# utiasDSL/upright

Measured on AMD Instinct MI355X. Metric: batched MPC solves/sec + ms/SQP-iter, Thing 1-obj horizon=20, 1/2/4/8 GPU, higher is better.
Workload: dtype f64

## Files before the change

### __graft_entry__.py

```python
import os
import subprocess
import sys
from pathlib import Path

ROOT = Path(__file__).resolve().parent
CSRC = ROOT / "upright_amd" / "csrc"
LIB = ROOT / "upright_amd" / "libupright_mi.so"


def _newer(srcs, out):
    return (not out.exists()) or any(s.stat().st_mtime > out.stat().st_mtime for s in srcs)


def n_qp3_parts():
    import re

    m = re.search(r"#define\s+UPR_QP3_NPARTS\s+(\d+)", (CSRC / "upr_qp3_list.h").read_text())
    return int(m.group(1))


def build_engine(out=None, extra_flags=()):
    from concurrent.futures import ThreadPoolExecutor

    out = Path(out) if out else LIB
# ... 42 lines not shown
        subprocess.check_call(["g++", "-O2", "-std=c++17", "-fPIC", "-shared", "-Wno-unknown-pragmas", "-o", str(bal_out), str(bal_src)])
    mar_src = ROOT / "tests" / "emu" / "upr_margin_emu.cpp"
    mar_out = ROOT / "tests" / "emu" / "libupr_margin_emu.so"
    if _newer(srcs + [mar_src], mar_out):
        subprocess.check_call(["g++", "-O2", "-std=c++17", "-fPIC", "-shared", "-Wno-unknown-pragmas", "-o", str(mar_out), str(mar_src)])
    grp_src = ROOT / "tests" / "emu" / "upr_group_margin_emu.cpp"
    grp_out = ROOT / "tests" / "emu" / "libupr_group_margin_emu.so"
    if _newer(srcs + [grp_src], grp_out):
        subprocess.check_call(["g++", "-O2", "-std=c++17", "-fPIC", "-shared", "-Wno-unknown-pragmas", "-o", str(grp_out), str(grp_src)])
    spd_src = ROOT / "tests" / "emu" / "upr_speed_emu.cpp"
    spd_out = ROOT / "tests" / "emu" / "libupr_speed_emu.so"
    if _newer(srcs + [spd_src], spd_out):
        subprocess.check_call(["g++", "-O2", "-std=c++17", "-fPIC", "-shared", "-Wno-unknown-pragmas", "-o", str(spd_out), str(spd_src)])
    spd_fma = ROOT / "tests" / "emu" / "libupr_speed_emu_fma.so"
    if has_fma and _newer(srcs + [spd_src], spd_fma):
        subprocess.check_call(["g++", "-O2", "-mfma", "-ffp-contract=fast", "-std=c++17", "-fPIC", "-shared", "-Wno-unknown-pragmas", "-o", str(spd_fma), str(spd_src)])
    pac_src = ROOT / "tests" / "emu" / "upr_pathacc_emu.cpp"
    pac_out = ROOT / "tests" / "emu" / "libupr_pathacc_emu.so"
    if _newer(srcs + [pac_src], pac_out):
        subprocess.check_call(["g++", "-O2", "-std=c++17", "-fPIC", "-shared", "-Wno-unknown-pragmas", "-o", str(pac_out), str(pac_src)])
    pac_fma = ROOT / "tests" / "emu" / "libupr_pathacc_emu_fma.so"
    if has_fma and _newer(srcs + [pac_src], pac_fma):
        subprocess.check_call(["g++", "-O2", "-mfma", "-ffp-contract=fast", "-std=c++17", "-fPIC", "-shared", "-Wno-unknown-pragmas", "-o", str(pac_fma), str(pac_src)])
    sys.path.insert(0, str(ROOT))
    import upright_amd
    from upright_amd import _capi

    _capi.lib()


def smoke():
    import json

    import numpy as np

    sys.path.insert(0, str(ROOT))
    from oracle.oracle import Oracle
    from upright_amd.engine import BatchMPC
    from upright_amd.problem import thing_problem
    from upright_amd.sampling import level_tray_states, stationary_guess, waypoints_for

    arr = json.load(open(ROOT / "tests" / "golden" / "arrangements.json"))["pink_bottle"]
    P = thing_problem(arr)
    B = 4
    x0 = level_tray_states(B, seed=3)
    way = waypoints_for(P, x0)
# ... 21 lines not shown
```

### upright_amd/csrc/upr_api.hip

```cpp
#include <hip/hip_runtime.h>
#include <hip/hiprtc.h>

#include <dlfcn.h>
#include <sys/stat.h>
#include <unistd.h>

#include <algorithm>
#include <chrono>
#include <fstream>
#include <map>
#include <mutex>
#include <sstream>
#include <cmath>
#include <cstdio>
#include <cstdlib>
#include <cstring>
#include <string>
#include <vector>

#include "upr_common.h"
#include "upr_kin.h"
#include "upr_linearize.h"
#include "upr_linearize2.h"
#include "upr_linesearch.h"
#include "upr_qp.h"
#include "upr_qp2.h"
#include "upr_qp3.h"
#include "upr_qp3_list.h"
#include "upr_qp3_launch.h"
#include "upr_qp_select.h"
#include "upr_launch_select.h"
#include "upr_value.h"
#include "upr_balance.h"
#include "upr_margin.h"
#include "upr_speed.h"
#include "upr_pathacc.h"
#include "upr_iface.h"

namespace {

thread_local std::string g_err;

int fail(const std::string& msg) {
    g_err = msg;
    return 1;
}

#define UPR_HIP(call)                                                                                 \
    do {                                                                                              \
        hipError_t e_ = (call);                                                                       \
        if (e_ != hipSuccess) return fail(std::string(#call) + ": " + hipGetErrorString(e_) + " (upr_api.hip:" + std::to_string(__LINE__) + ")"); \
    } while (0)

// ... 67 lines not shown
    if (threadIdx.x == 0) done[b] = 0;
}

__global__ void evaluate_kernel(const upr_problem* P, upr_dims d, int B, const double* tsol, const double* xs,
                                const double* us, const double* t, int t_stride, double* x_out, double* u_out) {
    int b = blockIdx.x;
    const int N = d.N, nx = d.nx, nu = d.nu;
    const double tau = t[(size_t)b * t_stride];
    for (int i = threadIdx.x; i < nx; i += blockDim.x)
        upr_interp(d, P->dt, tsol[b], xs + (size_t)b * (N + 1) * nx, us + (size_t)b * N * nu, tau, i, 0, x_out + (size_t)b * nx + i, nullptr);
    for (int i = threadIdx.x; i < nu; i += blockDim.x)
        upr_interp(d, P->dt, tsol[b], xs + (size_t)b * (N + 1) * nx, us + (size_t)b * N * nu, tau, 0, i, nullptr, u_out + (size_t)b * nu + i);
}

struct upr_fb_src {
    int kind;
    long k_base; int k_stride;
    long lji_base; int lji_stride;
    long lfi_base; int lfi_stride;
    long lsi_base; int lsi_stride;
    int lsi_sb;
};

template <int NEM, int NFM>
__global__ void feedback_kernel(const upr_problem* P, upr_dims d, upr_fb_src src, const double* ws, const double* lin,
                                const double* Df, const double* stats, double* fb) {
    const int b = blockIdx.x;
    const int N = d.N, nq = d.nq, nx = d.nx, nu = d.nu, ne = d.ne, nfc = d.nfc, nf = d.nf;
    const double* w = ws + (size_t)b * d.ws_stride;
    double* out = fb + (size_t)b * N * nu * nx;
    if (stats[(size_t)b * UPR_NSTATS + 2] == 2.0) {
        for (int e = threadIdx.x; e < N * nu * nx; e += blockDim.x) out[e] = 0.0;
        return;
    }
    for (int e = threadIdx.x; e < N * nq * nx; e += blockDim.x) {
        const int k = e / (nq * nx), j = (e % (nq * nx)) / nx, c = e % nx;
        double v;
        if (src.kind == 3) v = w[src.k_base + (long)k * src.k_stride + j * nx + c];
        else {
            const double* V = w + src.k_base + (long)k * src.k_stride;
            const double* Lji = w + src.lji_base + (long)k * src.lji_stride;
            v = 0.0;
            for (int m = j; m < nq; ++m) v += Lji[m * nq + j] * V[m * nx + c];
        }
        out[((size_t)k * nu + j) * nx + c] = -v;
    }
    const double* Dfb = Df + (size_t)b * ne * nfc;
    for (int e = threadIdx.x; e < N * nx; e += blockDim.x) {
        const int k = e / nx, c = e % nx;
        const double* Ck = lin + ((size_t)b * (N + 1) + k) * d.lin_stride + d.lin_gx;
        const double* Lsi = w + src.lsi_base + (long)k * src.lsi_stride;
        const double* Lfi = w + src.lfi_base + (long)k * src.lfi_stride;
        double t1[NEM], t2[NEM], t3[NFM];
        const int sb = src.lsi_sb;
        for (int r = 0; r < ne; ++r) { const int b0 = (r / sb) * sb; const double* Lb = Lsi + (b0 / sb) * sb * sb; double v = 0.0; for (int m = b0; m <= r; ++m) v += Lb[(r - b0) * sb + (m - b0)] * Ck[m * nx + c]; t1[r] = v; }
        for (int r = 0; r < ne; ++r) { const int b0 = (r / sb) * sb; const double* Lb = Lsi + (b0 / sb) * sb * sb; double v = 0.0; for (int m = r; m < b0 + sb; ++m) v += Lb[(m - b0) * sb + (r - b0)] * t1[m]; t2[r] = v; }
        for (int i = 0; i < nfc; ++i) { double v = 0.0; for (int r = 0; r < ne; ++r) v += Dfb[r * nfc + i] * t2[r]; t3[i] = v; }
        for (int ci = 0; ci < d.nc; ++ci) {
            if (nf == 3) {
                const double* Bk = Lfi + 9 * ci; const double* x3 = t3 + 3 * ci;
                double y[3], z[3];
                for (int a = 0; a < 3; ++a) { double v = 0.0; for (int b2 = 0; b2 <= a; ++b2) v += Bk[3 * a + b2] * x3[b2]; y[a] = v; }
                for (int a = 0; a < 3; ++a) { double v = 0.0; for (int b2 = a; b2 < 3; ++b2) v += Bk[3 * b2 + a] * y[b2]; z[a] = v; }
                for (int a = 0; a < 3; ++a) out[((size_t)k * nu + nq + 3 * ci + a) * nx + c] = -z[a];
            } else {
                const double lf = Lfi[ci];
                out[((size_t)k * nu + nq + ci) * nx + c] = -lf * lf * t3[ci];
            }
        }
    }
}

__global__ void evaluate_policy_kernel(const upr_problem* P, upr_dims d, int B, const double* tsol, const double* xs,
                                       const double* us, const double* fb, const double* t, const double* x_obs,
                                       double* x_out, double* u_out) {
    const int b = blockIdx.x;
    const int N = d.N, nx = d.nx, nu = d.nu;
    const double* X = xs + (size_t)b * (N + 1) * nx; const double* U = us + (size_t)b * N * nu;
    const double* K = fb + (size_t)b * N * nu * nx; const double* xo = x_obs + (size_t)b * nx;
    double s = (t[b] - tsol[b]) / P->dt;
    if (s < 0.0) s = 0.0;
    for (int i = threadIdx.x; i < nx; i += blockDim.x)
        upr_interp(d, P->dt, tsol[b], X, U, t[b], i, 0, x_out + (size_t)b * nx + i, nullptr);
    for (int i = threadIdx.x; i < nu; i += blockDim.x) {
        double v = 0.0;
        if (s <= N) {
            int j = (int)s; if (j > N - 1) j = N - 1;
            const double a = (s >= N - 1) ? 0.0 : s - j;
            const int j1 = (j + 1 < N) ? j + 1 : N - 1;
            double v0 = U[j * nu + i], v1 = U[j1 * nu + i];
            for (int c = 0; c < nx; ++c) {
                v0 += K[((size_t)j * nu + i) * nx + c] * (xo[c] - X[j * nx + c]);
                if (a > 0.0) v1 += K[((size_t)j1 * nu + i) * nx + c] * (xo[c] - X[j1 * nx + c]);
            }
            v = (1.0 - a) * v0 + a * v1;
        }
        u_out[(size_t)b * nu + i] = v;
    }
}

}

#define UPR_ENTER(h) do { if (!(h)) return fail("null batch"); if ((h)->device >= 0) UPR_HIP(hipSetDevice((h)->device)); } while (0)

struct upr_jit_kernel {
    hipModule_t mod = nullptr;
    hipFunction_t fn = nullptr;
    size_t lds = 0, ws = 0;
    int nt = 256;
    std::string cfg;
    upr_fb_src fb{};
};

struct upr_qp_sel : upr_qp_choice {
    int (*launch)(struct upr_batch*, const upr_qp_args&) = nullptr;
    upr_jit_kernel* jit = nullptr;
    upr_fb_src fb{};
};

struct upr_lin_sel : upr_lin_choice {
    const void* kern = nullptr;
    char name[128] = "";
};
// ... 12 lines not shown
struct upr_stats_snapshot {
    std::vector<double> stats; std::vector<unsigned char> keys;
};
}

struct upr_batch {
    upr_problem P;
    upr_dims d;
    int B = 0;
    int device = -1;
    hipStream_t stream = nullptr;
    upr_problem* dP = nullptr;
    double *body_params = nullptr, *way_p = nullptr, *way_q = nullptr, *t0 = nullptr, *x0 = nullptr;
    double *xs = nullptr, *us = nullptr, *xs_prev = nullptr, *us_prev = nullptr, *tprev = nullptr;
    double *lin = nullptr, *Df = nullptr, *ws = nullptr, *stats = nullptr;
    int *done = nullptr;
    bool has_prev = false;
    unsigned char* iter_key = nullptr;
    int* order = nullptr;
    bool order_on = true, order_valid = false;
    double* prof = nullptr;
    double *ev_t = nullptr, *ev_xo = nullptr, *ev_x = nullptr, *ev_u = nullptr;
    double* kkt = nullptr;
    double *fb = nullptr, *xs_lin = nullptr;
    double *dyn0 = nullptr, *pflag = nullptr;
    std::vector<double> hdyn0, hdyn_prev;
    double* pin = nullptr;
    hipGraphExec_t tick_exec = nullptr;
    unsigned long long tick_sig = 0;
    int tick_steady = 0;
    int tick_graph_on = -1;
    long long tick_replays = 0;
    int nxf = 0;
    bool guess_set = false;
    int sqp_iters_next = 0;
    double last_ms = 0.0;
    upr_qp_sel qp;
    upr_lin_sel lin_sel;
    upr_ls_sel ls_sel;
    int lin_blocks_last = -1;
    bool ls_launched = false;
    int timing = 0;
    unsigned timing_qp_count = 0;
    double k_ms[3] = {0, 0, 0};
    int k_launches[3] = {0, 0, 0};
    std::vector<double> hDf;
// ... 358 lines not shown
    void stop() { if (on) (void)hipEventRecord(h->ev_pool[idx + 1], h->stream); }
};

int vf_alloc(upr_batch* h) {
    if (h->vf_P) return 0;
    const size_t B = (size_t)h->B, n1 = (size_t)h->d.N + 1, nx = (size_t)h->d.nx;
    if (dev_alloc(&h->vf_P, B * n1 * nx * nx) || dev_alloc(&h->vf_p, B * n1 * nx) || dev_alloc(&h->vf_J, B * n1) || dev_alloc(&h->vf_X, B * n1 * nx) || dev_alloc(&h->vf_t0, B) ||
        dev_alloc(&h->vf_nu, B * (size_t)h->d.N * (size_t)h->d.ne)) return 1;
    UPR_HIP(hipEventCreate(&h->vf_ev[0])); UPR_HIP(hipEventCreate(&h->vf_ev[1]));
    return 0;
}
upr_vf_args make_vf_args(upr_batch* h) {
    upr_vf_args A;
    A.P = h->dP; A.d = h->d; A.xs = h->xs; A.us = h->us; A.lin = h->lin; A.Df = h->Df; A.ws = h->ws;
    const upr_qp_sel& q = h->qp;
    A.mult = q.exported ? h->kkt : h->ws; A.mult_stride = q.stride;
    A.o_pi = q.o_pi; A.o_nu = q.o_nu; A.o_lam = q.o_lam; A.o_t = q.o_t; A.o_sig = q.o_sig; A.o_tau = q.o_tau; A.o_gam = q.o_gam;
    A.Pk = h->vf_P; A.pk = h->vf_p; A.J = h->vf_J; A.X = h->vf_X; A.nu_out = h->vf_nu;
    return A;
}
size_t vf_lds_bytes(const upr_batch* h) { return (size_t)upr_vf_lds_layout(h->d).total * sizeof(double); }
hipError_t vf_raise_lds_limit() { return hipFuncSetAttribute((const void*)upr_value_kernel, hipFuncAttributeMaxDynamicSharedMemorySize, 160 * 1024); }

int advance_impl(upr_batch* h) {
    const upr_dims& d = h->d;
    if (h->vf_state) h->vf_state = 2;
    if (!h->guess_set) {
        hipLaunchKernelGGL(prepare_kernel, dim3(h->B), dim3(256), 0, h->stream, h->dP, d, h->B, h->has_prev ? 1 : 0, h->tprev,
                           h->xs_prev, h->us_prev, h->t0, h->x0, h->xs, h->us, h->stats, h->done);
        UPR_HIP(hipGetLastError());
    } else {
        UPR_HIP(hipMemsetAsync(h->stats, 0, sizeof(double) * h->B * UPR_NSTATS, h->stream));
        UPR_HIP(hipMemsetAsync(h->done, 0, sizeof(int) * h->B, h->stream));
        h->guess_set = false;
    }
    const int sqp_iters = h->sqp_iters_next > 0 ? h->sqp_iters_next : h->P.sqp_iters;
    h->sqp_iters_next = 0;
    for (int it = 0; it < sqp_iters; ++it) {
        { KernelTimer T(h, 0); if (launch_linearize(h, traj_lin_args(h))) return 1; T.stop(); }
        {
            upr_qp_args Q = make_qp_args(h);
            if (h->fb && h->qp.fb_fused && it == sqp_iters - 1) Q.fb = h->fb;
            if (h->order_on && h->order_valid) Q.order = h->order;
            if (h->vf_track && it == sqp_iters - 1 && h->qp.exported) { Q.kkt = h->kkt; Q.kkt_stride = h->qp.stride; }
            KernelTimer T(h, 1); if (launch_qp(h, Q)) return 1; T.stop();
        }
        if (h->vf_track && it == sqp_iters - 1) {
            const bool timed = h->timing != 0;
            if (timed) UPR_HIP(hipEventRecord(h->vf_ev[0], h->stream));
            hipLaunchKernelGGL(upr_value_kernel, dim3(h->B), dim3(UPR_VF_NT), vf_lds_bytes(h), h->stream, make_vf_args(h));
            UPR_HIP(hipGetLastError());
            if (timed) { UPR_HIP(hipEventRecord(h->vf_ev[1], h->stream)); h->vf_ms_pending = true; }
            UPR_HIP(hipMemcpyAsync(h->vf_t0, h->t0, sizeof(double) * h->B, hipMemcpyDeviceToDevice, h->stream));
            h->vf_state = 1; h->vf_tracked = true;
        }
        upr_ls_args L;
        L.P = h->dP; L.d = d; L.xs = h->xs; L.us = h->us; L.x0 = h->x0; L.t0 = h->t0; L.body_params = h->body_params;
        L.way_p = h->way_p; L.way_q = upr_has_orientation_cost(&h->P) ? h->way_q : nullptr; L.lin = h->lin; L.ws = h->ws; L.stats = h->stats; L.done = h->done; L.iter = it; L.dyn = h->dyn0; L.pflag = h->pflag;
        if (h->order_on) { L.order_out = h->order; L.iter_key = h->iter_key; }
        if (it == sqp_iters - 1) { L.xs_prev = h->xs_prev; L.us_prev = h->us_prev; L.tprev = h->tprev; }
        { KernelTimer T(h, 2); if (launch_linesearch(h, L)) return 1; T.stop(); }
        if (h->order_on) h->order_valid = true;
    }
    if (h->fb && !(h->qp.fb_fused && sqp_iters > 0)) {
        if (h->qp.fb.kind == 0) return fail("feedback gains: the selected QP kernel names no source for them");
        if (d.ne <= 6 && d.nfc <= 12) hipLaunchKernelGGL((feedback_kernel<6, 12>), dim3(h->B), dim3(256), 0, h->stream, h->dP, d, h->qp.fb, h->ws, h->lin, h->Df, h->stats, h->fb);
        else hipLaunchKernelGGL((feedback_kernel<6 * UPR_MAX_BODIES, 3 * UPR_MAX_CONTACTS>), dim3(h->B), dim3(256), 0, h->stream, h->dP, d, h->qp.fb, h->ws, h->lin, h->Df, h->stats, h->fb);
        UPR_HIP(hipGetLastError());
    }
    h->hdyn_prev = h->hdyn0;
    if (sqp_iters <= 0) {
        UPR_HIP(hipMemcpyAsync(h->xs_prev, h->xs, sizeof(double) * h->B * (d.N + 1) * d.nx, hipMemcpyDeviceToDevice, h->stream));
        UPR_HIP(hipMemcpyAsync(h->us_prev, h->us, sizeof(double) * h->B * d.N * d.nu, hipMemcpyDeviceToDevice, h->stream));
        UPR_HIP(hipMemcpyAsync(h->tprev, h->t0, sizeof(double) * h->B, hipMemcpyDeviceToDevice, h->stream));
    }
    h->has_prev = true;
    return 0;
}

enum { BAL_MU_NONE = 0, BAL_MU_SCENARIO = 1, BAL_MU_CONTACT = 2 };
enum { BAL_RHO = 0, BAL_MARGIN = 1, BAL_MARGIN_GROUPS = 2, BAL_SPEED = 3, BAL_PATHACC = 4 };
struct bal_request {
    const char* who = "";
    const char* needs = "";
    bool plan = false; int n = 0; const double* x = nullptr;
    int n_scen = 0; const double* params = nullptr; bool per = false;
    int scale = BAL_MU_NONE; const double* mu_scale = nullptr;
    int quantity = BAL_RHO; double kappa_max = 0.0; int n_grp = 1; const unsigned* group_mask = nullptr; const double* mu_base = nullptr;
    double s_max = 0.0; double* limit = nullptr;
    double d_max = 0.0, speed = 1.0;
    double* out = nullptr;
    double *kappa_lo = nullptr, *z = nullptr, *y = nullptr; int* iters = nullptr; double* worst = nullptr; int* worst_knot = nullptr;
// ... 235 lines not shown
    UPR_HIP(hipMemcpy(out, dout, sizeof(double) * n * 5 * P->nc, hipMemcpyDeviceToHost));
    return 0;
}

upr_batch* upr_batch_create(const upr_problem* P, int B, const double* body_params, const double* way_p) {
    if (check_problem(P)) return nullptr;
    if (B < 1) { fail("B must be >= 1"); return nullptr; }
    if (need_device()) return nullptr;
    upr_batch* h = new upr_batch();
    if (hipGetDevice(&h->device) != hipSuccess) { fail("hipGetDevice failed"); delete h; return nullptr; }
    h->P = *P; h->d = upr_make_dims(P); h->B = B;
    h->nxf = (int)upr_iface_width(h->d.nx, P->n_dyn);
    h->hdyn0.assign((size_t)B * upr_iface_dyn_width(P->n_dyn), 0.0); h->hdyn_prev = h->hdyn0;
    const upr_dims& d = h->d;
    if (d.nx > UPR_LPK) { fail("nx exceeds the 32 tangent lanes of the linearisation kernel"); delete h; return nullptr; }
    {
        upr_qp_knobs k;
        if (const char* e = getenv("UPR_QP_KERNEL")) k.qp_kernel = atoi(e);
        if (const char* e = getenv("UPR_QP_GENERIC")) k.qp_generic = atoi(e) != 0;
        if (const char* e = getenv("UPR_QP3_JIT")) k.qp3_jit = atoi(e);
        if (const char* e = getenv("UPR_QP_NT")) { k.qp_nt_set = true; k.qp_nt = atoi(e); }
        if (const char* e = getenv("UPR_QP_GENERIC_NT")) { k.generic_nt_set = true; k.generic_nt = atoi(e); }
        if (const char* e = getenv("UPR_JIT_NT")) k.jit_nt = atoi(e);
        if (const char* e = getenv("UPR_FB_FUSED")) k.fb_fused = atoi(e) != 0;
        upr_qp_sel& s = h->qp;
        static_cast<upr_qp_choice&>(s) = upr_qp_plan(*P, d, k);
        if (s.source == UPR_QP_FROM_RUN_TIME && s.structure == UPR_QP_STRUCT_PRODUCTION && jit_get(s.cfg, s.nt, &s.jit) != 0) {
            static_cast<upr_qp_choice&>(s) = upr_qp_plan(*P, d, k, false);
            fprintf(stderr, "libupright_mi: %s -- using the %s kernel instead\n", g_err.c_str(), s.structure == UPR_QP_STRUCT_SECOND ? "second-structure" : "generic");
        }
        qp_resolve(s, *P, d);
        h->d.ws_stride = s.ws_stride;
    }
    {
        upr_lin_knobs kl; upr_ls_knobs ks;
        if (const char* e = getenv("UPR_LIN_MFMA")) kl.mfma = atoi(e) != 0;
        if (const char* e = getenv("UPR_LIN2")) kl.lin2 = atoi(e) != 0;
        if (const char* e = getenv("UPR_LIN_OCC")) kl.occ = atoi(e);
        if (const char* e = getenv("UPR_LIN_ROW_PASSES")) kl.row_passes = atoi(e);
        if (const char* e = getenv("UPR_LS_STAGE_FULL")) ks.stage_full = atoi(e);
        static_cast<upr_lin_choice&>(h->lin_sel) = upr_lin_plan(*P, d, kl);
        static_cast<upr_ls_choice&>(h->ls_sel) = upr_ls_plan(*P, d, ks);
        h->lin_sel.kern = (P->nq == 6) ? lin_kernel<6>(h->lin_sel) : lin_kernel<9>(h->lin_sel);
        h->ls_sel.kern = (P->nq == 6) ? ls_kernel<6>(h->ls_sel) : ls_kernel<9>(h->ls_sel);
        upr_ls_name(h->ls_sel, h->ls_sel.name, sizeof(h->ls_sel.name));
        if (!h->lin_sel.kern || !h->ls_sel.kern) { fail("the planned linearisation / line-search form is not an instantiation of upr_launch_select.h's lists"); delete h; return nullptr; }
    }
    if (const char* e = getenv("UPR_QP_ORDER")) h->order_on = atoi(e) != 0;
    {
        const char* e = getenv("UPR_BAL_FORM");
        h->bal.L = upr_bal_layout(d.nb, d.nc, d.nf);
        h->bal.lds = (size_t)h->bal.L.total * sizeof(double);
        h->bal.form = (upr_bal_lane_form(d.nb) && !(e && atoi(e) == 0)) ? BAL_LANE : BAL_WAVE;
    }
    auto bad = [&]() { upr_batch_destroy(h); return (upr_batch*)nullptr; };
    if (hipStreamCreate(&h->stream) != hipSuccess) { fail("hipStreamCreate failed"); return bad(); }
    if (hipMalloc((void**)&h->dP, sizeof(upr_problem)) != hipSuccess) { fail("hipMalloc failed"); return bad(); }
    hipMemcpy(h->dP, P, sizeof(upr_problem), hipMemcpyHostToDevice);
    const size_t n1 = d.N + 1;
    if (dev_alloc(&h->body_params, (size_t)B * d.nb * 10) || dev_alloc(&h->way_p, (size_t)B * P->n_way * 3) || dev_alloc(&h->way_q, (size_t)B * P->n_way * 4) ||
        dev_alloc(&h->t0, (((size_t)B + 1) & ~(size_t)1) + (size_t)B * d.nx + (size_t)B * upr_iface_dyn_width(P->n_dyn)) || dev_alloc(&h->xs, (size_t)B * n1 * d.nx) || dev_alloc(&h->us, (size_t)B * d.N * d.nu) ||
        dev_alloc(&h->xs_prev, (size_t)B * n1 * d.nx) || dev_alloc(&h->us_prev, (size_t)B * d.N * d.nu) || dev_alloc(&h->tprev, B) ||
        dev_alloc(&h->lin, (size_t)B * n1 * d.lin_stride) || dev_alloc(&h->Df, (size_t)B * d.ne * d.nfc) ||
        dev_alloc(&h->ws, (size_t)B * d.ws_stride) || dev_alloc(&h->stats, (size_t)B * UPR_NSTATS) || dev_alloc(&h->done, B) || dev_alloc(&h->order, B) || dev_alloc(&h->iter_key, ((size_t)B + 3) & ~(size_t)3) ||
        (P->use_feedback_policy && dev_alloc(&h->fb, (size_t)B * d.N * d.nu * d.nx)) ||
        (P->n_dyn && dev_alloc(&h->pflag, B)))
        return bad();
    h->x0 = h->t0 + (((size_t)B + 1) & ~(size_t)1);
    if (P->n_dyn) h->dyn0 = h->x0 + (size_t)B * d.nx;
    hipMemcpy(h->body_params, body_params, sizeof(double) * B * d.nb * 10, hipMemcpyHostToDevice);
    hipMemcpy(h->way_p, way_p, sizeof(double) * B * P->n_way * 3, hipMemcpyHostToDevice);
    {
        std::vector<double> qi((size_t)B * P->n_way * 4, 0.0);
        for (size_t i = 3; i < qi.size(); i += 4) qi[i] = 1.0;
        hipMemcpy(h->way_q, qi.data(), sizeof(double) * qi.size(), hipMemcpyHostToDevice);
    }
    h->hDf.assign((size_t)B * d.ne * d.nfc, 0.0);
    std::vector<double> unit(d.nfc), Fw(6 * d.nb);
    const double scale = 1.0 / std::sqrt(6.0 * d.nb);
    for (int b = 0; b < B; ++b) {
        const double* bp = body_params + (size_t)b * d.nb * 10;
        for (int j = 0; j < d.nfc; ++j) {
            std::fill(unit.begin(), unit.end(), 0.0);
            unit[j] = 1.0;
            upr_object_wrenches(P, bp, unit.data(), Fw.data());
            for (int bb = 0; bb < d.nb; ++bb)
                for (int r = 0; r < 6; ++r) h->hDf[((size_t)b * d.ne + 6 * bb + r) * d.nfc + j] = -scale * Fw[6 * bb + r] / bp[10 * bb];
        }
// ... 86 lines not shown
int upr_batch_advance(upr_batch* h) {
    UPR_ENTER(h);
    auto t0 = std::chrono::steady_clock::now();
    if (advance_impl(h)) return 1;
    UPR_HIP(hipStreamSynchronize(h->stream));
    h->last_ms = std::chrono::duration<double, std::milli>(std::chrono::steady_clock::now() - t0).count();
    return 0;
}

static int get_solution_core(upr_batch* h, double* ts, double* xs, double* us) {
    const upr_dims& d = h->d;
    UPR_HIP(hipStreamSynchronize(h->stream));
    if (ts) {
        std::vector<double> t0(h->B);
        UPR_HIP(hipMemcpy(t0.data(), h->t0, sizeof(double) * h->B, hipMemcpyDeviceToHost));
        for (int b = 0; b < h->B; ++b) for (int k = 0; k <= d.N; ++k) ts[(size_t)b * (d.N + 1) + k] = t0[b] + k * h->P.dt;
    }
    if (xs) UPR_HIP(hipMemcpy(xs, h->xs, sizeof(double) * h->B * (d.N + 1) * d.nx, hipMemcpyDeviceToHost));
    if (us) UPR_HIP(hipMemcpy(us, h->us, sizeof(double) * h->B * d.N * d.nu, hipMemcpyDeviceToHost));
    return 0;
}

static int evaluate_core(upr_batch* h, const double* t, int t_stride, bool policy, const double* x_obs, double* x_out, double* u_out) {
    if (policy && !h->fb) return fail("upr_batch_evaluate_policy: the batch was created with use_feedback_policy = 0");
    const upr_dims& d = h->d;
    if (eval_scratch(h)) return 1;
    std::vector<double> tt(h->B);
    instance_times(h->B, t, t_stride, tt.data());
    UPR_HIP(hipMemcpyAsync(h->ev_t, tt.data(), sizeof(double) * h->B, hipMemcpyHostToDevice, h->stream));
    if (policy) {
        UPR_HIP(hipMemcpyAsync(h->ev_xo, x_obs, sizeof(double) * h->B * d.nx, hipMemcpyHostToDevice, h->stream));
        hipLaunchKernelGGL(evaluate_policy_kernel, dim3(h->B), dim3(64), 0, h->stream, h->dP, d, h->B, h->tprev, h->xs_prev, h->us_prev, h->fb, h->ev_t, h->ev_xo, h->ev_x, h->ev_u);
    } else hipLaunchKernelGGL(evaluate_kernel, dim3(h->B), dim3(64), 0, h->stream, h->dP, d, h->B, h->tprev, h->xs_prev, h->us_prev, h->ev_t, 1, h->ev_x, h->ev_u);
    UPR_HIP(hipGetLastError());
    UPR_HIP(hipMemcpyAsync(x_out, h->ev_x, sizeof(double) * h->B * d.nx, hipMemcpyDeviceToHost, h->stream));
    UPR_HIP(hipMemcpyAsync(u_out, h->ev_u, sizeof(double) * h->B * d.nu, hipMemcpyDeviceToHost, h->stream));
    UPR_HIP(hipStreamSynchronize(h->stream));
    return 0;
}

static int get_feedback_core(upr_batch* h, double* K) {
    if (!h->fb) return fail("upr_batch_get_feedback: the batch was created with use_feedback_policy = 0");
    const upr_dims& d = h->d;
    UPR_HIP(hipStreamSynchronize(h->stream));
    UPR_HIP(hipMemcpy(K, h->fb, sizeof(double) * h->B * d.N * d.nu * d.nx, hipMemcpyDeviceToHost));
    return 0;
}

double upr_batch_last_solve_ms(const upr_batch* h) { return h ? h->last_ms : 0.0; }

const char* upr_batch_qp_kernel_name(const upr_batch* h) { return h ? h->qp.name : ""; }

const char* upr_batch_ls_kernel_name(upr_batch* h) {
    if (!h || !h->ls_launched) return "";
    return h->ls_sel.name;
}

const char* upr_batch_lin_kernel_name(upr_batch* h) {
    if (!h || h->lin_blocks_last < 0) return "";
    upr_lin_name(h->lin_sel, h->lin_blocks_last, h->lin_sel.name, sizeof(h->lin_sel.name));
    return h->lin_sel.name;
}

int upr_batch_hold_stats(upr_batch* h, int restore) {
    UPR_ENTER(h);
    UPR_HIP(hipStreamSynchronize(h->stream));
    if (!restore) return snapshot_take(h, h->held);
    if (h->held.stats.empty()) return fail("upr_batch_hold_stats: nothing held on this handle");
    if (snapshot_put_back(h, h->held)) return 1;
    h->held = upr_stats_snapshot();
    return 0;
}

int upr_batch_get_stats(upr_batch* h, double* stats) {
    UPR_ENTER(h);
    UPR_HIP(hipStreamSynchronize(h->stream));
    UPR_HIP(hipMemcpy(stats, h->stats, sizeof(double) * h->B * UPR_NSTATS, hipMemcpyDeviceToHost));
    return 0;
}

static int linearize_points_impl(upr_batch* h, int n, const int* inst, const double* t, const double* x, const double* u, std::vector<double>& rec, double* ee) {
    const upr_dims& d = h->d;
    const size_t nd = upr_iface_dyn_width(h->P.n_dyn);
    point_upload pts;
    if (pts.up(h, n, inst, t)) return 1;
    std::vector<double> xr, dyn;
    if (h->P.n_dyn) {
        xr.resize((size_t)n * d.nx); dyn.resize((size_t)n * nd);
        upr_iface_split(d.nx, h->P.n_dyn, x, (size_t)n, xr.data(), dyn.data());
        x = xr.data();
    }
// ... 58 lines not shown
}

int upr_batch_state_rows(upr_batch* h, int n, const int* inst, const double* t, const double* x, double* dd, double* dq) {
    UPR_ENTER(h);
    const upr_dims& d = h->d;
    if (d.no == 0) return fail("upr_batch_state_rows: the problem has no state rows");
    if (n <= 0) return 0;
    return state_rows_impl(h, n, inst, t, x, d.no, dd, dq);
}

int upr_batch_eq_input_jacobian(upr_batch* h, int inst, double* gu) {
    UPR_ENTER(h);
    if (inst < 0 || inst >= h->B) return fail("instance index out of range");
    const upr_dims& d = h->d;
    for (int r = 0; r < d.ne; ++r) {
        for (int j = 0; j < d.nq; ++j) gu[(size_t)r * d.nu + j] = 0.0;
        for (int j = 0; j < d.nfc; ++j) gu[(size_t)r * d.nu + d.nq + j] = h->hDf[((size_t)inst * d.ne + r) * d.nfc + j];
    }
    return 0;
}

static int kkt_launch(upr_batch* h) {
    if (h->qp.exported && !h->kkt && dev_alloc(&h->kkt, (size_t)h->B * h->qp.stride)) return 1;
    if (launch_linearize(h, traj_lin_args(h))) return 1;
    upr_qp_args A = make_qp_args(h);
    if (h->qp.exported) { A.kkt = h->kkt; A.kkt_stride = h->qp.stride; }
    return launch_qp(h, A);
}

static int qp_step_core(upr_batch* h, double* dxs, double* dus) {
    const upr_dims& d = h->d;
    if (launch_linearize(h, traj_lin_args(h))) return 1;
    if (launch_qp(h, make_qp_args(h))) return 1;
    UPR_HIP(hipStreamSynchronize(h->stream));
    std::vector<double> ws((size_t)h->B * d.ws_stride);
    UPR_HIP(hipMemcpy(ws.data(), h->ws, sizeof(double) * ws.size(), hipMemcpyDeviceToHost));
    for (int b = 0; b < h->B; ++b) {
        const double* w = ws.data() + (size_t)b * d.ws_stride;
        if (dxs) std::memcpy(dxs + (size_t)b * (d.N + 1) * d.nx, w + d.ws_dx, sizeof(double) * (d.N + 1) * d.nx);
        if (dus) std::memcpy(dus + (size_t)b * d.N * d.nu, w + d.ws_du, sizeof(double) * d.N * d.nu);
    }
    return 0;
}

static int qp_kkt_core(upr_batch* h, double* dxs, double* dus, double* pi, double* nu, double* yN, double* lam, int* ni_out) {
    const upr_dims& d = h->d;
    if (ni_out) *ni_out = d.ni_stage;
    const upr_qp_sel& sel = h->qp;
    if (kkt_launch(h)) return 1;
    UPR_HIP(hipStreamSynchronize(h->stream));
    std::vector<double> ws((size_t)h->B * d.ws_stride), kk;
    UPR_HIP(hipMemcpy(ws.data(), h->ws, sizeof(double) * ws.size(), hipMemcpyDeviceToHost));
    if (sel.exported) { kk.resize((size_t)h->B * sel.stride); UPR_HIP(hipMemcpy(kk.data(), h->kkt, sizeof(double) * kk.size(), hipMemcpyDeviceToHost)); }
    const int n1 = d.N + 1;
// ... 424 lines not shown
}

int upr_batch_tick(upr_batch* h, const double* t, int t_stride, const double* x, double* x_out, double* u_out, double* stats_out) {
    UPR_ENTER(h);
    if (!t || !x || !x_out || !u_out) return fail("upr_batch_tick: null argument");
    if (h->vf_state) h->vf_state = 2;
    const upr_dims& d = h->d;
    const size_t B = (size_t)h->B, nx = (size_t)d.nx, nu = (size_t)d.nu, ndyn = upr_iface_dyn_width(h->P.n_dyn);
    if (eval_scratch(h)) return 1;
    const size_t Bt = (B + 1) & ~(size_t)1;
    const size_t n_in = Bt + B * nx + B * ndyn, n_out = B * nx + B * nu + B * UPR_NSTATS;
    if (!h->pin) {
        UPR_HIP(hipHostMalloc((void**)&h->pin, sizeof(double) * (n_in + n_out), hipHostMallocDefault));
    }
    double* pt = h->pin; double* px = pt + Bt; double* pd = px + B * nx;
    double* ox = h->pin + n_in; double* ou = ox + B * nx; double* os = ou + B * nu;
    instance_times(h->B, t, t_stride, pt);
    upr_iface_split(d.nx, h->P.n_dyn, x, B, px, ndyn ? pd : nullptr);
    if (ndyn) std::memcpy(h->hdyn0.data(), pd, sizeof(double) * B * ndyn);
    auto t0c = std::chrono::steady_clock::now();
    auto enqueue = [&]() -> int {
        UPR_HIP(hipMemcpyAsync(h->t0, pt, sizeof(double) * n_in, hipMemcpyHostToDevice, h->stream));
        if (advance_impl(h)) return 1;
        if (h->fb) hipLaunchKernelGGL(evaluate_policy_kernel, dim3(h->B), dim3(64), 0, h->stream, h->dP, d, h->B, h->tprev, h->xs_prev, h->us_prev, h->fb, h->t0, h->x0, h->ev_x, h->ev_u);
        else hipLaunchKernelGGL(evaluate_kernel, dim3(h->B), dim3(64), 0, h->stream, h->dP, d, h->B, h->tprev, h->xs_prev, h->us_prev, h->t0, 1, h->ev_x, h->ev_u);
        UPR_HIP(hipGetLastError());
        UPR_HIP(hipMemcpyAsync(ox, h->ev_x, sizeof(double) * (B * nx + B * nu), hipMemcpyDeviceToHost, h->stream));
        if (stats_out) UPR_HIP(hipMemcpyAsync(os, h->stats, sizeof(double) * B * UPR_NSTATS, hipMemcpyDeviceToHost, h->stream));
        return 0;
    };
    if (h->tick_graph_on < 0) { const char* e = getenv("UPR_TICK_GRAPH"); h->tick_graph_on = (e && atoi(e) == 0) ? 0 : 1; }
    const int sqp_now = h->sqp_iters_next > 0 ? h->sqp_iters_next : h->P.sqp_iters;
    unsigned long long sig = 1469598103934665603ull;
    for (unsigned long long v : {(unsigned long long)h->has_prev, (unsigned long long)h->guess_set, (unsigned long long)sqp_now, (unsigned long long)(h->order_on && h->order_valid),
                                 (unsigned long long)(h->fb != nullptr), (unsigned long long)h->qp.fb_fused, (unsigned long long)h->timing, (unsigned long long)(stats_out != nullptr),
                                 (unsigned long long)h->qp.structure, (unsigned long long)h->qp.source, (unsigned long long)h->qp.nt, (unsigned long long)(uintptr_t)h->pin,
                                 (unsigned long long)(uintptr_t)h->prof ,
                                 (unsigned long long)h->vf_track }) { sig ^= v; sig *= 1099511628211ull; }
    const bool steady = h->tick_graph_on && !h->timing && h->has_prev && !h->guess_set && h->sqp_iters_next == 0 && (!h->order_on || h->order_valid);
    if (steady && h->tick_exec && sig == h->tick_sig) {
        UPR_HIP(hipGraphLaunch(h->tick_exec, h->stream));
        h->hdyn_prev = h->hdyn0;
        if (h->vf_track && sqp_now > 0) { h->vf_state = 1; h->vf_tracked = true; }
        ++h->tick_replays;
    } else {
        if (h->tick_exec && sig != h->tick_sig) { (void)hipGraphExecDestroy(h->tick_exec); h->tick_exec = nullptr; h->tick_steady = 0; }
        h->tick_steady = (steady && sig == h->tick_sig) ? h->tick_steady + 1 : 0;
        h->tick_sig = sig;
        if (steady && h->tick_steady >= 2 && !h->tick_exec) {
            hipGraph_t g = nullptr;
            UPR_HIP(hipStreamBeginCapture(h->stream, hipStreamCaptureModeThreadLocal));
            const int rc = enqueue();
            const hipError_t ec = hipStreamEndCapture(h->stream, &g);
            if (rc || ec != hipSuccess || !g) { if (g) (void)hipGraphDestroy(g); h->tick_graph_on = 0; if (rc) return 1; if (enqueue()) return 1; }
            else {
                const hipError_t ei = hipGraphInstantiate(&h->tick_exec, g, nullptr, nullptr, 0);
                (void)hipGraphDestroy(g);
                if (ei != hipSuccess) { h->tick_exec = nullptr; h->tick_graph_on = 0; if (enqueue()) return 1; }
                else UPR_HIP(hipGraphLaunch(h->tick_exec, h->stream));
            }
        } else if (enqueue()) return 1;
    }
    UPR_HIP(hipStreamSynchronize(h->stream));
    h->last_ms = std::chrono::duration<double, std::milli>(std::chrono::steady_clock::now() - t0c).count();
    upr_iface_join(d.nx, h->P.n_dyn, ox, pd, B, x_out);
// ... 64 lines not shown
```

Measured before the change: 544,000.

## Compute feedback gains lazily from QP factors instead of gathering full array

Adds an on-demand feedback-gain mode: after each solve the full N×nu×nx gain array is no longer materialized. The policy evaluation instead rebuilds gains for the one or two needed knots straight from the QP workspace factors, using shared memory. A small state machine tracks whether gains live as factors or as an array, and gathers them only when a caller needs the full array or the factors are about to be overwritten. This removes the per-tick feedback kernel or fused write, at the cost of more state-management complexity and recomputing gains during policy evaluation.

```diff
diff --git a/__graft_entry__.py b/__graft_entry__.py
--- a/__graft_entry__.py
+++ b/__graft_entry__.py
@@ -88,6 +88,10 @@
     pac_fma = ROOT / "tests" / "emu" / "libupr_pathacc_emu_fma.so"
     if has_fma and _newer(srcs + [pac_src], pac_fma):
         subprocess.check_call(["g++", "-O2", "-mfma", "-ffp-contract=fast", "-std=c++17", "-fPIC", "-shared", "-Wno-unknown-pragmas", "-o", str(pac_fma), str(pac_src)])
+    fbs_src = ROOT / "tests" / "emu" / "upr_fb_state_emu.cpp"
+    fbs_out = ROOT / "tests" / "emu" / "libupr_fb_state_emu.so"
+    if _newer(srcs + [fbs_src], fbs_out):
+        subprocess.check_call(["g++", "-O2", "-std=c++17", "-fPIC", "-shared", "-o", str(fbs_out), str(fbs_src)])
     sys.path.insert(0, str(ROOT))
     import upright_amd
     from upright_amd import _capi
diff --git a/upright_amd/csrc/upr_api.hip b/upright_amd/csrc/upr_api.hip
--- a/upright_amd/csrc/upr_api.hip
+++ b/upright_amd/csrc/upr_api.hip
@@ -29,6 +29,7 @@
 #include "upr_qp3_list.h"
 #include "upr_qp3_launch.h"
 #include "upr_qp_select.h"
+#include "upr_fb_state.h"
 #include "upr_launch_select.h"
 #include "upr_value.h"
 #include "upr_balance.h"
@@ -142,11 +143,44 @@
     int lsi_sb;
 };
 
+__device__ inline double fb_jerk_entry(const upr_dims& d, const upr_fb_src& src, const double* w, int k, int j, int c) {
+    const int nq = d.nq, nx = d.nx;
+    if (src.kind == 3) return w[src.k_base + (long)k * src.k_stride + j * nx + c];
+    const double* V = w + src.k_base + (long)k * src.k_stride;
+    const double* Lji = w + src.lji_base + (long)k * src.lji_stride;
+    double v = 0.0;
+    for (int m = j; m < nq; ++m) v += Lji[m * nq + j] * V[m * nx + c];
+    return v;
+}
+template <int NEM, int NFM>
+__device__ inline void fb_force_column(const upr_dims& d, const upr_fb_src& src, const double* w, const double* Ck, const double* Dfb, int k, int c, double* out) {
+    const int nq = d.nq, nx = d.nx, ne = d.ne, nfc = d.nfc, nf = d.nf;
+    const double* Lsi = w + src.lsi_base + (long)k * src.lsi_stride;
+    const double* Lfi = w + src.lfi_base + (long)k * src.lfi_stride;
+    double t1[NEM], t2[NEM], t3[NFM];
+    const int sb = src.lsi_sb;
+    for (int r = 0; r < ne; ++r) { const int b0 = (r / sb) * sb; const double* Lb = Lsi + (b0 / sb) * sb * sb; double v = 0.0; for (int m = b0; m <= r; ++m) v += Lb[(r - b0) * sb + (m - b0)] * Ck[m * nx + c]; t1[r] = v; }
+    for (int r = 0; r < ne; ++r) { const int b0 = (r / sb) * sb; const double* Lb = Lsi + (b0 / sb) * sb * sb; double v = 0.0; for (int m = r; m < b0 + sb; ++m) v += Lb[(m - b0) * sb + (r - b0)] * t1[m]; t2[r] = v; }
+    for (int i = 0; i < nfc; ++i) { double v = 0.0; for (int r = 0; r < ne; ++r) v += Dfb[r * nfc + i] * t2[r]; t3[i] = v; }
+    for (int ci = 0; ci < d.nc; ++ci) {
+        if (nf == 3) {
+            const double* Bk = Lfi + 9 * ci; const double* x3 = t3 + 3 * ci;
+            double y[3], z[3];
+            for (int a = 0; a < 3; ++a) { double v = 0.0; for (int b2 = 0; b2 <= a; ++b2) v += Bk[3 * a + b2] * x3[b2]; y[a] = v; }
+            for (int a = 0; a < 3; ++a) { double v = 0.0; for (int b2 = a; b2 < 3; ++b2) v += Bk[3 * b2 + a] * y[b2]; z[a] = v; }
+            for (int a = 0; a < 3; ++a) out[(size_t)(nq + 3 * ci + a) * nx + c] = -z[a];
+        } else {
+            const double lf = Lfi[ci];
+            out[(size_t)(nq + ci) * nx + c] = -lf * lf * t3[ci];
+        }
+    }
+}
+
 template <int NEM, int NFM>
 __global__ void feedback_kernel(const upr_problem* P, upr_dims d, upr_fb_src src, const double* ws, const double* lin,
                                 const double* Df, const double* stats, double* fb) {
     const int b = blockIdx.x;
-    const int N = d.N, nq = d.nq, nx = d.nx, nu = d.nu, ne = d.ne, nfc = d.nfc, nf = d.nf;
+    const int N = d.N, nq = d.nq, nx = d.nx, nu = d.nu, ne = d.ne, nfc = d.nfc;
     const double* w = ws + (size_t)b * d.ws_stride;
     double* out = fb + (size_t)b * N * nu * nx;
     if (stats[(size_t)b * UPR_NSTATS + 2] == 2.0) {
@@ -155,39 +189,13 @@
     }
     for (int e = threadIdx.x; e < N * nq * nx; e += blockDim.x) {
         const int k = e / (nq * nx), j = (e % (nq * nx)) / nx, c = e % nx;
-        double v;
-        if (src.kind == 3) v = w[src.k_base + (long)k * src.k_stride + j * nx + c];
-        else {
-            const double* V = w + src.k_base + (long)k * src.k_stride;
-            const double* Lji = w + src.lji_base + (long)k * src.lji_stride;
-            v = 0.0;
-            for (int m = j; m < nq; ++m) v += Lji[m * nq + j] * V[m * nx + c];
-        }
-        out[((size_t)k * nu + j) * nx + c] = -v;
+        out[((size_t)k * nu + j) * nx + c] = -fb_jerk_entry(d, src, w, k, j, c);
     }
     const double* Dfb = Df + (size_t)b * ne * nfc;
     for (int e = threadIdx.x; e < N * nx; e += blockDim.x) {
         const int k = e / nx, c = e % nx;
         const double* Ck = lin + ((size_t)b * (N + 1) + k) * d.lin_stride + d.lin_gx;
-        const double* Lsi = w + src.lsi_base + (long)k * src.lsi_stride;
-        const double* Lfi = w + src.lfi_base + (long)k * src.lfi_stride;
-        double t1[NEM], t2[NEM], t3[NFM];
-        const int sb = src.lsi_sb;
-        for (int r = 0; r < ne; ++r) { const int b0 = (r / sb) * sb; const double* Lb = Lsi + (b0 / sb) * sb * sb; double v = 0.0; for (int m = b0; m <= r; ++m) v += Lb[(r - b0) * sb + (m - b0)] * Ck[m * nx + c]; t1[r] = v; }
-        for (int r = 0; r < ne; ++r) { const int b0 = (r / sb) * sb; const double* Lb = Lsi + (b0 / sb) * sb * sb; double v = 0.0; for (int m = r; m < b0 + sb; ++m) v += Lb[(m - b0) * sb + (r - b0)] * t1[m]; t2[r] = v; }
-        for (int i = 0; i < nfc; ++i) { double v = 0.0; for (int r = 0; r < ne; ++r) v += Dfb[r * nfc + i] * t2[r]; t3[i] = v; }
-        for (int ci = 0; ci < d.nc; ++ci) {
-            if (nf == 3) {
-                const double* Bk = Lfi + 9 * ci; const double* x3 = t3 + 3 * ci;
-                double y[3], z[3];
-                for (int a = 0; a < 3; ++a) { double v = 0.0; for (int b2 = 0; b2 <= a; ++b2) v += Bk[3 * a + b2] * x3[b2]; y[a] = v; }
-                for (int a = 0; a < 3; ++a) { double v = 0.0; for (int b2 = a; b2 < 3; ++b2) v += Bk[3 * b2 + a] * y[b2]; z[a] = v; }
-                for (int a = 0; a < 3; ++a) out[((size_t)k * nu + nq + 3 * ci + a) * nx + c] = -z[a];
-            } else {
-                const double lf = Lfi[ci];
-                out[((size_t)k * nu + nq + ci) * nx + c] = -lf * lf * t3[ci];
-            }
-        }
+        fb_force_column<NEM, NFM>(d, src, w, Ck, Dfb, k, c, out + (size_t)k * nu * nx);
     }
 }
 
@@ -219,6 +227,52 @@
     }
 }
 
+template <int NEM, int NFM>
+__global__ void evaluate_policy_factors_kernel(const upr_problem* P, upr_dims d, int B, const double* tsol, const double* xs,
+                                               const double* us, upr_fb_src src, const double* ws, const double* lin, const double* Df,
+                                               const double* stats, const double* t, const double* x_obs, double* x_out, double* u_out) {
+    extern __shared__ double fb_lds[];
+    const int b = blockIdx.x;
+    const int N = d.N, nq = d.nq, nx = d.nx, nu = d.nu, ne = d.ne, nfc = d.nfc;
+    const double* X = xs + (size_t)b * (N + 1) * nx; const double* U = us + (size_t)b * N * nu;
+    const double* xo = x_obs + (size_t)b * nx;
+    double s = (t[b] - tsol[b]) / P->dt;
+    if (s < 0.0) s = 0.0;
+    for (int i = threadIdx.x; i < nx; i += blockDim.x)
+        upr_interp(d, P->dt, tsol[b], X, U, t[b], i, 0, x_out + (size_t)b * nx + i, nullptr);
+    int j = (int)s; if (j > N - 1) j = N - 1;
+    const double a = (s >= N - 1) ? 0.0 : s - j;
+    const int j1 = (j + 1 < N) ? j + 1 : N - 1;
+    const bool inside = s <= N, policy = stats[(size_t)b * UPR_NSTATS + 2] != 2.0;
+    if (inside && policy) {
+        const double* w = ws + (size_t)b * d.ws_stride;
+        const double* Dfb = Df + (size_t)b * ne * nfc;
+        const int nk = a > 0.0 ? 2 : 1;
+        for (int q = 0; q < nk; ++q) {
+            const int k = q ? j1 : j;
+            double* G = fb_lds + (size_t)q * nu * nx;
+            for (int e = threadIdx.x; e < nq * nx; e += blockDim.x) G[e] = -fb_jerk_entry(d, src, w, k, e / nx, e % nx);
+            const double* Ck = lin + ((size_t)b * (N + 1) + k) * d.lin_stride + d.lin_gx;
+            for (int c = threadIdx.x; c < nx; c += blockDim.x) fb_force_column<NEM, NFM>(d, src, w, Ck, Dfb, k, c, G);
+        }
+    }
+    __syncthreads();
+    const double* K0 = fb_lds; const double* K1 = fb_lds + (size_t)nu * nx;
+    for (int i = threadIdx.x; i < nu; i += blockDim.x) {
+        double v = 0.0;
+        if (inside) {
+            double v0 = U[j * nu + i], v1 = U[j1 * nu + i];
+            if (policy) for (int c = 0; c < nx; ++c) {
+                v0 += K0[(size_t)i * nx + c] * (xo[c] - X[j * nx + c]);
+                if (a > 0.0) v1 += K1[(size_t)i * nx + c] * (xo[c] - X[j1 * nx + c]);
+            }
+            v = (1.0 - a) * v0 + a * v1;
+        }
+        u_out[(size_t)b * nu + i] = v;
+    }
+}
+static_assert(2 * UPR_MAX_NU * UPR_MAX_NX * sizeof(double) <= 64 * 1024, "two knots of gains in the LDS a kernel gets without asking");
+
 }
 
 #define UPR_ENTER(h) do { if (!(h)) return fail("null batch"); if ((h)->device >= 0) UPR_HIP(hipSetDevice((h)->device)); } while (0)
@@ -277,6 +331,8 @@
     double* prof = nullptr;
     double *ev_t = nullptr, *ev_xo = nullptr, *ev_x = nullptr, *ev_u = nullptr;
     double* kkt = nullptr;
+    bool fb_on = false;
+    upr_fb_track fbt;
     double *fb = nullptr, *xs_lin = nullptr;
     double *dyn0 = nullptr, *pflag = nullptr;
     std::vector<double> hdyn0, hdyn_prev;
@@ -681,9 +737,46 @@
 size_t vf_lds_bytes(const upr_batch* h) { return (size_t)upr_vf_lds_layout(h->d).total * sizeof(double); }
 hipError_t vf_raise_lds_limit() { return hipFuncSetAttribute((const void*)upr_value_kernel, hipFuncAttributeMaxDynamicSharedMemorySize, 160 * 1024); }
 
+int fb_gather(upr_batch* h) {
+    const upr_dims& d = h->d;
+    if (!h->fb && dev_alloc(&h->fb, (size_t)h->B * d.N * d.nu * d.nx)) return 1;
+    if (h->qp.fb.kind == 0) return fail("feedback gains: the selected QP kernel names no source for them");
+    if (d.ne <= 6 && d.nfc <= 12) hipLaunchKernelGGL((feedback_kernel<6, 12>), dim3(h->B), dim3(256), 0, h->stream, h->dP, d, h->qp.fb, h->ws, h->lin, h->Df, h->stats, h->fb);
+    else hipLaunchKernelGGL((feedback_kernel<6 * UPR_MAX_BODIES, 3 * UPR_MAX_CONTACTS>), dim3(h->B), dim3(256), 0, h->stream, h->dP, d, h->qp.fb, h->ws, h->lin, h->Df, h->stats, h->fb);
+    UPR_HIP(hipGetLastError());
+    return 0;
+}
+int fb_keep(upr_batch* h) {
+    if (!h->fb_on || !upr_fb_must_gather(h->fbt)) return 0;
+    if (fb_gather(h)) return 1;
+    h->fbt.state = upr_fb_after_gather(h->fbt);
+    return 0;
+}
+int launch_policy(upr_batch* h, const double* t, const double* x_obs) {
+    const upr_dims& d = h->d;
+    if (upr_fb_policy_from_factors(h->fbt.state)) {
+        if (h->qp.fb.kind == 0) return fail("feedback gains: the selected QP kernel names no source for them");
+        const size_t lds = sizeof(double) * 2 * d.nu * d.nx;
+        if (d.ne <= 6 && d.nfc <= 12) hipLaunchKernelGGL((evaluate_policy_factors_kernel<6, 12>), dim3(h->B), dim3(64), lds, h->stream, h->dP, d, h->B, h->tprev, h->xs_prev, h->us_prev, h->qp.fb, h->ws, h->lin, h->Df, h->stats, t, x_obs, h->ev_x, h->ev_u);
+        else hipLaunchKernelGGL((evaluate_policy_factors_kernel<6 * UPR_MAX_BODIES, 3 * UPR_MAX_CONTACTS>), dim3(h->B), dim3(64), lds, h->stream, h->dP, d, h->B, h->tprev, h->xs_prev, h->us_prev, h->qp.fb, h->ws, h->lin, h->Df, h->stats, t, x_obs, h->ev_x, h->ev_u);
+    } else {
+        if (!h->fb && dev_alloc(&h->fb, (size_t)h->B * d.N * d.nu * d.nx)) return 1;
+        hipLaunchKernelGGL(evaluate_policy_kernel, dim3(h->B), dim3(64), 0, h->stream, h->dP, d, h->B, h->tprev, h->xs_prev, h->us_prev, h->fb, t, x_obs, h->ev_x, h->ev_u);
+    }
+    UPR_HIP(hipGetLastError());
+    return 0;
+}
+
 int advance_impl(upr_batch* h) {
     const upr_dims& d = h->d;
     if (h->vf_state) h->vf_state = 2;
+    const int sqp_iters = h->sqp_iters_next > 0 ? h->sqp_iters_next : h->P.sqp_iters;
+    h->sqp_iters_next = 0;
+    upr_fb_advance fba;
+    if (h->fb_on) {
+        fba = upr_fb_on_advance(h->fbt, sqp_iters, h->qp.fb_fused);
+        if (fba.gather_before && fb_keep(h)) return 1;
+    }
     if (!h->guess_set) {
         hipLaunchKernelGGL(prepare_kernel, dim3(h->B), dim3(256), 0, h->stream, h->dP, d, h->B, h->has_prev ? 1 : 0, h->tprev,
                            h->xs_prev, h->us_prev, h->t0, h->x0, h->xs, h->us, h->stats, h->done);
@@ -693,13 +786,11 @@
         UPR_HIP(hipMemsetAsync(h->done, 0, sizeof(int) * h->B, h->stream));
         h->guess_set = false;
     }
-    const int sqp_iters = h->sqp_iters_next > 0 ? h->sqp_iters_next : h->P.sqp_iters;
-    h->sqp_iters_next = 0;
     for (int it = 0; it < sqp_iters; ++it) {
         { KernelTimer T(h, 0); if (launch_linearize(h, traj_lin_args(h))) return 1; T.stop(); }
         {
             upr_qp_args Q = make_qp_args(h);
-            if (h->fb && h->qp.fb_fused && it == sqp_iters - 1) Q.fb = h->fb;
+            if (fba.kernel_writes && it == sqp_iters - 1) Q.fb = h->fb;
             if (h->order_on && h->order_valid) Q.order = h->order;
             if (h->vf_track && it == sqp_iters - 1 && h->qp.exported) { Q.kkt = h->kkt; Q.kkt_stride = h->qp.stride; }
             KernelTimer T(h, 1); if (launch_qp(h, Q)) return 1; T.stop();
@@ -721,12 +812,8 @@
         { KernelTimer T(h, 2); if (launch_linesearch(h, L)) return 1; T.stop(); }
         if (h->order_on) h->order_valid = true;
     }
-    if (h->fb && !(h->qp.fb_fused && sqp_iters > 0)) {
-        if (h->qp.fb.kind == 0) return fail("feedback gains: the selected QP kernel names no source for them");
-        if (d.ne <= 6 && d.nfc <= 12) hipLaunchKernelGGL((feedback_kernel<6, 12>), dim3(h->B), dim3(256), 0, h->stream, h->dP, d, h->qp.fb, h->ws, h->lin, h->Df, h->stats, h->fb);
-        else hipLaunchKernelGGL((feedback_kernel<6 * UPR_MAX_BODIES, 3 * UPR_MAX_CONTACTS>), dim3(h->B), dim3(256), 0, h->stream, h->dP, d, h->qp.fb, h->ws, h->lin, h->Df, h->stats, h->fb);
-        UPR_HIP(hipGetLastError());
-    }
+    if (fba.gather_after && fb_gather(h)) return 1;
+    if (h->fb_on) h->fbt.state = fba.state;
     h->hdyn_prev = h->hdyn0;
     if (sqp_iters <= 0) {
         UPR_HIP(hipMemcpyAsync(h->xs_prev, h->xs, sizeof(double) * h->B * (d.N + 1) * d.nx, hipMemcpyDeviceToDevice, h->stream));
@@ -1008,7 +1095,8 @@
         if (const char* e = getenv("UPR_QP_NT")) { k.qp_nt_set = true; k.qp_nt = atoi(e); }
         if (const char* e = getenv("UPR_QP_GENERIC_NT")) { k.generic_nt_set = true; k.generic_nt = atoi(e); }
         if (const char* e = getenv("UPR_JIT_NT")) k.jit_nt = atoi(e);
-        if (const char* e = getenv("UPR_FB_FUSED")) k.fb_fused = atoi(e) != 0;
+        if (const char* e = getenv("UPR_FB_FUSED")) { k.fb_fused = atoi(e) != 0; h->fbt.mode = UPR_FB_EAGER; }
+        h->fb_on = P->use_feedback_policy != 0;
         upr_qp_sel& s = h->qp;
         static_cast<upr_qp_choice&>(s) = upr_qp_plan(*P, d, k);
         if (s.source == UPR_QP_FROM_RUN_TIME && s.structure == UPR_QP_STRUCT_PRODUCTION && jit_get(s.cfg, s.nt, &s.jit) != 0) {
@@ -1049,7 +1137,7 @@
         dev_alloc(&h->xs_prev, (size_t)B * n1 * d.nx) || dev_alloc(&h->us_prev, (size_t)B * d.N * d.nu) || dev_alloc(&h->tprev, B) ||
         dev_alloc(&h->lin, (size_t)B * n1 * d.lin_stride) || dev_alloc(&h->Df, (size_t)B * d.ne * d.nfc) ||
         dev_alloc(&h->ws, (size_t)B * d.ws_stride) || dev_alloc(&h->stats, (size_t)B * UPR_NSTATS) || dev_alloc(&h->done, B) || dev_alloc(&h->order, B) || dev_alloc(&h->iter_key, ((size_t)B + 3) & ~(size_t)3) ||
-        (P->use_feedback_policy && dev_alloc(&h->fb, (size_t)B * d.N * d.nu * d.nx)) ||
+        (h->fb_on && h->fbt.mode == UPR_FB_EAGER && dev_alloc(&h->fb, (size_t)B * d.N * d.nu * d.nx)) ||
         (P->n_dyn && dev_alloc(&h->pflag, B)))
         return bad();
     h->x0 = h->t0 + (((size_t)B + 1) & ~(size_t)1);
@@ -1182,7 +1270,7 @@
 }
 
 static int evaluate_core(upr_batch* h, const double* t, int t_stride, bool policy, const double* x_obs, double* x_out, double* u_out) {
-    if (policy && !h->fb) return fail("upr_batch_evaluate_policy: the batch was created with use_feedback_policy = 0");
+    if (policy && !h->fb_on) return fail("upr_batch_evaluate_policy: the batch was created with use_feedback_policy = 0");
     const upr_dims& d = h->d;
     if (eval_scratch(h)) return 1;
     std::vector<double> tt(h->B);
@@ -1190,7 +1278,7 @@
     UPR_HIP(hipMemcpyAsync(h->ev_t, tt.data(), sizeof(double) * h->B, hipMemcpyHostToDevice, h->stream));
     if (policy) {
         UPR_HIP(hipMemcpyAsync(h->ev_xo, x_obs, sizeof(double) * h->B * d.nx, hipMemcpyHostToDevice, h->stream));
-        hipLaunchKernelGGL(evaluate_policy_kernel, dim3(h->B), dim3(64), 0, h->stream, h->dP, d, h->B, h->tprev, h->xs_prev, h->us_prev, h->fb, h->ev_t, h->ev_xo, h->ev_x, h->ev_u);
+        if (launch_policy(h, h->ev_t, h->ev_xo)) return 1;
     } else hipLaunchKernelGGL(evaluate_kernel, dim3(h->B), dim3(64), 0, h->stream, h->dP, d, h->B, h->tprev, h->xs_prev, h->us_prev, h->ev_t, 1, h->ev_x, h->ev_u);
     UPR_HIP(hipGetLastError());
     UPR_HIP(hipMemcpyAsync(x_out, h->ev_x, sizeof(double) * h->B * d.nx, hipMemcpyDeviceToHost, h->stream));
@@ -1200,8 +1288,10 @@
 }
 
 static int get_feedback_core(upr_batch* h, double* K) {
-    if (!h->fb) return fail("upr_batch_get_feedback: the batch was created with use_feedback_policy = 0");
-    const upr_dims& d = h->d;
+    if (!h->fb_on) return fail("upr_batch_get_feedback: the batch was created with use_feedback_policy = 0");
+    const upr_dims& d = h->d;
+    if (fb_keep(h)) return 1;
+    if (!h->fb && dev_alloc(&h->fb, (size_t)h->B * d.N * d.nu * d.nx)) return 1;
     UPR_HIP(hipStreamSynchronize(h->stream));
     UPR_HIP(hipMemcpy(K, h->fb, sizeof(double) * h->B * d.N * d.nu * d.nx, hipMemcpyDeviceToHost));
     return 0;
@@ -1227,6 +1317,8 @@
     UPR_HIP(hipStreamSynchronize(h->stream));
     if (!restore) return snapshot_take(h, h->held);
     if (h->held.stats.empty()) return fail("upr_batch_hold_stats: nothing held on this handle");
+    if (fb_keep(h)) return 1;
+    UPR_HIP(hipStreamSynchronize(h->stream));
     if (snapshot_put_back(h, h->held)) return 1;
     h->held = upr_stats_snapshot();
     return 0;
@@ -1331,6 +1423,7 @@
 
 static int kkt_launch(upr_batch* h) {
     if (h->qp.exported && !h->kkt && dev_alloc(&h->kkt, (size_t)h->B * h->qp.stride)) return 1;
+    if (fb_keep(h)) return 1;
     if (launch_linearize(h, traj_lin_args(h))) return 1;
     upr_qp_args A = make_qp_args(h);
     if (h->qp.exported) { A.kkt = h->kkt; A.kkt_stride = h->qp.stride; }
@@ -1339,6 +1432,7 @@
 
 static int qp_step_core(upr_batch* h, double* dxs, double* dus) {
     const upr_dims& d = h->d;
+    if (fb_keep(h)) return 1;
     if (launch_linearize(h, traj_lin_args(h))) return 1;
     if (launch_qp(h, make_qp_args(h))) return 1;
     UPR_HIP(hipStreamSynchronize(h->stream));
@@ -1809,7 +1903,7 @@
     auto enqueue = [&]() -> int {
         UPR_HIP(hipMemcpyAsync(h->t0, pt, sizeof(double) * n_in, hipMemcpyHostToDevice, h->stream));
         if (advance_impl(h)) return 1;
-        if (h->fb) hipLaunchKernelGGL(evaluate_policy_kernel, dim3(h->B), dim3(64), 0, h->stream, h->dP, d, h->B, h->tprev, h->xs_prev, h->us_prev, h->fb, h->t0, h->x0, h->ev_x, h->ev_u);
+        if (h->fb_on) { if (launch_policy(h, h->t0, h->x0)) return 1; }
         else hipLaunchKernelGGL(evaluate_kernel, dim3(h->B), dim3(64), 0, h->stream, h->dP, d, h->B, h->tprev, h->xs_prev, h->us_prev, h->t0, 1, h->ev_x, h->ev_u);
         UPR_HIP(hipGetLastError());
         UPR_HIP(hipMemcpyAsync(ox, h->ev_x, sizeof(double) * (B * nx + B * nu), hipMemcpyDeviceToHost, h->stream));
@@ -1820,14 +1914,16 @@
     const int sqp_now = h->sqp_iters_next > 0 ? h->sqp_iters_next : h->P.sqp_iters;
     unsigned long long sig = 1469598103934665603ull;
     for (unsigned long long v : {(unsigned long long)h->has_prev, (unsigned long long)h->guess_set, (unsigned long long)sqp_now, (unsigned long long)(h->order_on && h->order_valid),
-                                 (unsigned long long)(h->fb != nullptr), (unsigned long long)h->qp.fb_fused, (unsigned long long)h->timing, (unsigned long long)(stats_out != nullptr),
+                                 (unsigned long long)h->fb_on, (unsigned long long)h->qp.fb_fused, (unsigned long long)h->fbt.mode , (unsigned long long)h->timing, (unsigned long long)(stats_out != nullptr),
                                  (unsigned long long)h->qp.structure, (unsigned long long)h->qp.source, (unsigned long long)h->qp.nt, (unsigned long long)(uintptr_t)h->pin,
                                  (unsigned long long)(uintptr_t)h->prof ,
                                  (unsigned long long)h->vf_track }) { sig ^= v; sig *= 1099511628211ull; }
-    const bool steady = h->tick_graph_on && !h->timing && h->has_prev && !h->guess_set && h->sqp_iters_next == 0 && (!h->order_on || h->order_valid);
+    const bool steady = h->tick_graph_on && !h->timing && h->has_prev && !h->guess_set && h->sqp_iters_next == 0 && (!h->order_on || h->order_valid) &&
+                        (!h->fb_on || upr_fb_capturable(h->fbt, sqp_now));
     if (steady && h->tick_exec && sig == h->tick_sig) {
         UPR_HIP(hipGraphLaunch(h->tick_exec, h->stream));
         h->hdyn_prev = h->hdyn0;
+        if (h->fb_on) h->fbt.state = upr_fb_on_replay(h->fbt, sqp_now, h->qp.fb_fused);
         if (h->vf_track && sqp_now > 0) { h->vf_state = 1; h->vf_tracked = true; }
         ++h->tick_replays;
     } else {
diff --git a/upright_amd/csrc/upr_fb_state.h b/upright_amd/csrc/upr_fb_state.h
--- /dev/null
+++ b/upright_amd/csrc/upr_fb_state.h
@@ -0,0 +1,39 @@
+#pragma once
+
+enum { UPR_FB_NONE = 0,
+       UPR_FB_FACTORS = 1,
+       UPR_FB_ARRAY = 2 };
+enum { UPR_FB_ON_DEMAND = 0,
+       UPR_FB_EAGER = 1 };
+
+struct upr_fb_track {
+    int mode = UPR_FB_ON_DEMAND;
+    int state = UPR_FB_NONE;
+};
+
+struct upr_fb_advance {
+    bool gather_before = false;
+    bool kernel_writes = false;
+    bool gather_after = false;
+    int state = UPR_FB_NONE;
+};
+static inline upr_fb_advance upr_fb_on_advance(const upr_fb_track& t, int qps, bool kernel_can_write) {
+    upr_fb_advance a;
+    if (t.mode == UPR_FB_EAGER) {
+        a.kernel_writes = kernel_can_write && qps > 0;
+        a.gather_after = !a.kernel_writes;
+        a.state = UPR_FB_ARRAY;
+        return a;
+    }
+    if (qps > 0) { a.state = UPR_FB_FACTORS; return a; }
+    a.gather_before = t.state == UPR_FB_FACTORS;
+    a.state = t.state == UPR_FB_FACTORS ? UPR_FB_ARRAY : t.state;
+    return a;
+}
+static inline int upr_fb_on_replay(const upr_fb_track& t, int qps, bool kernel_can_write) { return upr_fb_on_advance(t, qps, kernel_can_write).state; }
+static inline bool upr_fb_capturable(const upr_fb_track& t, int qps) {
+    return t.mode == UPR_FB_EAGER || (t.state == UPR_FB_FACTORS && qps > 0);
+}
+static inline bool upr_fb_policy_from_factors(int state) { return state == UPR_FB_FACTORS; }
+static inline bool upr_fb_must_gather(const upr_fb_track& t) { return t.state == UPR_FB_FACTORS; }
+static inline int upr_fb_after_gather(const upr_fb_track& t) { return t.state == UPR_FB_FACTORS ? UPR_FB_ARRAY : t.state; }
```

New measurement: 553,800 (median of 6 runs). +1.8%, better.
